# zivy/LSQRRecipes

Hardware: AMD Instinct MI355X
Metric: RANSAC hypotheses/sec + final-fit residual, 10M pts, 1/2/4/8 GPU (higher is better)
Workload: dtype f64; 1 GPU; PlaneParametersEstimator + RANSAC, 10000000 points, 50% outliers, delta=0.50 (BASELINE.json configs[1]); points=10000000, streams=4, world_size=1, collectives=none (single GPU), repeats=3

## Files before the change

### lsqrrecipes_amd/csrc/cells.h

```cpp
#pragma once
#include <hip/hip_runtime.h>
#include <stdint.h>

#include "models.h"

#pragma clang diagnostic ignored "-Winline-asm"

namespace lsqr {

constexpr int kCellPtsMin = 128;
constexpr uint32_t kGroupPad = 4, kCellPad = 16;
constexpr uint32_t kQueues = 32;
constexpr uint32_t kQueuePitch = 1088;

struct CellBox {
  float c[3];
  float h[3];
  float pad[2];
};

__device__ inline unsigned long long ord_u64(double v) {
  unsigned long long b;
  __builtin_memcpy(&b, &v, 8);
  return (b >> 63) ? ~b : (b | 0x8000000000000000ULL);
}
inline double ord_u64_inv(unsigned long long o) {
  unsigned long long b = (o >> 63) ? (o & 0x7FFFFFFFFFFFFFFFULL) : ~o;
  double v;
  memcpy(&v, &b, 8);
  return v;
}

struct BoundsRow {
  unsigned long long mn[3], mx[3], amax, nonfinite;
};
template <int D>
__global__ __launch_bounds__(256) void k_bounds(const double *__restrict__ data, size_t stride,
                                                size_t n, BoundsRow *__restrict__ rows) {
  unsigned long long mn[D], mx[D], am = 0, bad = 0;
  for (int d = 0; d < D; d++) mn[d] = ~0ULL, mx[d] = 0ULL;
  auto one = [&](const double(&x)[D]) {
    bool fin = true;
    for (int d = 0; d < D; d++) fin = fin && (fabs(x[d]) <= 1.7976931348623157e308);
    if (!fin) {
// ... 780 lines not shown
  static __device__ inline v2f value(const v2f *xs, const v2f *fp) {
    return M::filter_value(xs, fp);
  }
};
template <int D>
inline CellConsts cell_consts(const LineCell<D> *, const ModelConsts &mc) {
  const double u = 5.9604644775390625e-08, s3 = 1.7320508075688774;
  const double rc = 2.0 * mc.delta, cap = 4.0 * mc.delta_sq;
  const double eta = 1e-12 * 2.0 * mc.absmax;
  CellConsts cc;
  memset(&cc, 0, sizeof cc);
  cc.f[0] = f32_down_host(mc.delta_sq);
  cc.f[1] = f32_up_host(mc.delta_sq);
  cc.f[2] = f32_up_host(6.0 * u * (1.0 + 4.0 * u) * (1.0 + 1e-6));
  cc.f[3] = f32_up_host((u * rc + 2.0 * eta) * (1.0 + 1e-6));
  cc.f[4] = f32_up_host(2.0 * s3 * rc * (1.0 + 1e-6));
  cc.f[5] = f32_up_host(4.0 * u * cap * (1.0 + 1e-6));
  cc.f[6] = f32_down_host(0.25 * mc.delta / (6.0 * s3 * u) * (1.0 - 1e-6));
  cc.f[7] = f32_down_host(0.25 * mc.delta_sq * (1.0 - 1e-6));
  return cc;
}

template <int NB>
__device__ __forceinline__ void cells_filter_squares(float (&bc)[NB]) {
  const float tin = bc[NB - 2], tout = bc[NB - 1];
  const bool off = !(tout < __builtin_inff());
  const float a = tin > 0.0f ? (tin * tin) * 0.9999998f : 0.0f;
  const float c = (tout * tout) * 1.0000002f;
  const float band = c - a;
  bc[NB - 2] = off ? 0.0f : a;
  bc[NB - 1] = off ? __builtin_bit_cast(float, 0xFFFFFFFFu) : band;
}

template <class CM, int PP, bool LDSB, bool DUP = false>
__device__ __forceinline__ void cells_survivors(const v2f (&xs)[PP][4], const float (&bc)[CM::NB], float *s_bc,
                                                unsigned long long surv, const int lane,
                                                const double *__restrict__ sorted, const size_t ns, const size_t cell,
                                                const double *__restrict__ spg, const ModelConsts &mc,
                                                uint32_t &accv) {
  typedef typename CM::M M;
  constexpr int D = M::ND, NB = CM::NB, NV = CM::NV, SPD = M::SP, CP = 128 * PP;
  (void)D, (void)NV, (void)CP;
  if (LDSB && surv) {
    float4 w0, w1;
    if constexpr (DUP) {
      static_assert(LDSB && NB == 6 && NV == 4, "slots: fp0 fp1 fp3 fp3 | a a fp2 band");
      w0.x = bc[0], w0.y = bc[1], w0.z = bc[3], w0.w = bc[3];
      w1.x = bc[4], w1.y = bc[4], w1.z = bc[2], w1.w = bc[5];
    } else {
      w0.x = bc[0], w0.y = NB > 1 ? bc[1 < NB ? 1 : 0] : 0.0f, w0.z = NB > 2 ? bc[2 < NB ? 2 : 0] : 0.0f,
      w0.w = NB > 3 ? bc[3 < NB ? 3 : 0] : 0.0f;
      w1.x = NB > 4 ? bc[4 < NB ? 4 : 0] : 0.0f, w1.y = NB > 5 ? bc[5 < NB ? 5 : 0] : 0.0f,
      w1.z = NB > 6 ? bc[6 < NB ? 6 : 0] : 0.0f, w1.w = NB > 7 ? bc[7 < NB ? 7 : 0] : 0.0f;
    }
    ((float4 *)s_bc)[2 * lane] = w0;
    ((float4 *)s_bc)[2 * lane + 1] = w1;
  }
  while (surv) {
    const int b = __builtin_ctzll(surv);
    asm("s_bitset0_b64 %0, %1" : "+s"(surv) : "s"(b));
    v2f fp[NV], na;
    uint32_t band;
    if constexpr (DUP) {
      const float4 r0 = ((const float4 *)s_bc)[2 * b], r1 = ((const float4 *)s_bc)[2 * b + 1];
      fp[0].x = r0.x, fp[0].y = r0.x, fp[1].x = r0.y, fp[1].y = r0.y, fp[2].x = r1.z, fp[2].y = r1.z;
      fp[3].x = r0.z, fp[3].y = r0.w;
      na.x = -r1.x, na.y = -r1.y;
      band = __builtin_bit_cast(uint32_t, r1.w);
    } else if (LDSB) {
      static_assert(NB <= 8, "broadcast area holds 8 floats per lane");
      const float4 r0 = ((const float4 *)s_bc)[2 * b], r1 = ((const float4 *)s_bc)[2 * b + 1];
      const float rb[8] = {r0.x, r0.y, r0.z, r0.w, r1.x, r1.y, r1.z, r1.w};
// ... 2 lines not shown
      na.x = -rb[NB - 2], na.y = -rb[NB - 2];
      band = __builtin_bit_cast(uint32_t, rb[NB - 1]);
    } else {
#pragma unroll
      for (int k = 0; k < NV; k++) {
        float v = __builtin_bit_cast(
            float, __builtin_amdgcn_readlane(__builtin_bit_cast(int, bc[k]), b));
        fp[k].x = v;
        fp[k].y = v;
      }
      const float a = __builtin_bit_cast(float, __builtin_amdgcn_readlane(__builtin_bit_cast(int, bc[NB - 2]), b));
      na.x = -a, na.y = -a;
      band = (uint32_t)__builtin_amdgcn_readlane(__builtin_bit_cast(int, bc[NB - 1]), b);
    }
    unsigned long long in[2 * PP];
    uint32_t dmin = 0;
    v2f sv[PP];
#pragma unroll
    for (int p = 0; p < PP; p++) sv[p] = CM::value(xs[p], fp);
#pragma unroll
    for (int p = 0; p < PP; p++) {
      const v2f s = sv[p];
      const v2f d = __builtin_elementwise_fma(s, s, na);
      in[2 * p] = __ballot(d.x < 0.0f);
      in[2 * p + 1] = __ballot(d.y < 0.0f);
      typedef uint32_t v2u __attribute__((ext_vector_type(2)));
      const v2u du = __builtin_bit_cast(v2u, d);
      const uint32_t m = du.x < du.y ? du.x : du.y;
      dmin = p == 0 ? m : (m < dmin ? m : dmin);
    }
    const unsigned long long amb = __ballot(dmin <= band);
    if (amb) {
      const double *hp = spg + (size_t)b * SPD;
#pragma unroll
      for (int p = 0; p < PP; p++) {
        const size_t i0 = cell * CP + p * 128 + lane, i1 = i0 + 64;
        double r0[D], r1[D];
#pragma unroll
        for (int d = 0; d < D; d++) {
          r0[d] = i0 < ns ? sorted[i0 * D + d] : __builtin_nan("");
          r1[d] = i1 < ns ? sorted[i1 * D + d] : __builtin_nan("");
        }
        in[2 * p] = __ballot(M::agree(hp, r0, mc));
        in[2 * p + 1] = __ballot(M::agree(hp, r1, mc));
      }
    }
    uint32_t cnt = 0;
#pragma unroll
    for (int p = 0; p < 2 * PP; p++) cnt += (uint32_t)__builtin_popcountll(in[p]);
    asm volatile("s_mov_b32 m0, %2\n\tv_writelane_b32 %0, %1, m0"
                 : "+v"(accv)
                 : "s"(cnt), "s"(b)
                 : "m0");
  }
}

template <class CM, int PP>
__device__ __forceinline__ void cells_load(const double *__restrict__ sorted, const size_t ns, const size_t cell,
                                           const int lane, const double (&ctr)[3], v2f (&xs)[PP][4]) {
  constexpr int D = CM::M::ND, CP = 128 * PP;
#pragma unroll
  for (int p = 0; p < PP; p++) {
    const size_t i0 = cell * CP + p * 128 + lane, i1 = i0 + 64;
    const double *p0 = sorted + (i0 < ns ? i0 : 0) * D, *p1 = sorted + (i1 < ns ? i1 : 0) * D;
#pragma unroll
    for (int d = 0; d < 3; d++) {
// ... 323 lines not shown
  const uint32_t h = blockIdx.x * 256 + threadIdx.x;
  if (h >= cap) return;
  float row[ROW], row2[NR2 ? 4 * NR2 : 4];
  const float4 *r4 = (const float4 *)(rows + (size_t)(h < H ? h : 0) * ROW);
#pragma unroll
  for (int k = 0; k < NR4; k++) {
    const float4 v = r4[k];
    row[4 * k] = v.x, row[4 * k + 1] = v.y, row[4 * k + 2] = v.z, row[4 * k + 3] = v.w;
  }
  if constexpr (NR2 > 0) {
    const float4 *q4 = (const float4 *)(spf + (size_t)(h < H ? h : 0) * M::SPF + CM::ROW2_OFF);
#pragma unroll
    for (int k = 0; k < NR2; k++) {
      const float4 v = q4[k];
      row2[4 * k] = v.x, row2[4 * k + 1] = v.y, row2[4 * k + 2] = v.z, row2[4 * k + 3] = v.w;
    }
  }
  typename CM::Hyp hy;
  CM::prepare(row, row2, h < H, cc, hy);
  const HypWords<CM> hw = __builtin_bit_cast(HypWords<CM>, hy);
#pragma unroll
  for (int k = 0; k < NH4; k++)
    out[(size_t)h * NH4 + k] = make_float4(hw.w[4 * k], hw.w[4 * k + 1], hw.w[4 * k + 2], hw.w[4 * k + 3]);
}
template <class CM>
__device__ __forceinline__ typename CM::Hyp hyp_from(const float4 (&v)[HypWords<CM>::N4]) {
  HypWords<CM> hw;
#pragma unroll
  for (int k = 0; k < HypWords<CM>::N4; k++)
    hw.w[4 * k] = v[k].x, hw.w[4 * k + 1] = v[k].y, hw.w[4 * k + 2] = v[k].z, hw.w[4 * k + 3] = v[k].w;
  return __builtin_bit_cast(typename CM::Hyp, hw);
}

template <class CM, int PP, bool PREP = false, bool COUNT = false>
__global__ __launch_bounds__(256) void k_cells_bounds(const CellBox *__restrict__ boxes, uint32_t ncells,
                                                      size_t ns, const float *__restrict__ rows,
                                                      const float *__restrict__ spf, uint32_t H,
                                                      CellConsts cc, uint32_t cells_per_block,
                                                      uint32_t *__restrict__ ub,
                                                      unsigned long long *__restrict__ total,
                                                      uint32_t *__restrict__ ncells_out,
                                                      uint8_t *__restrict__ cnt, uint32_t gstride,
                                                      const uint32_t *__restrict__ h_dev, uint32_t h_off,
                                                      uint32_t box_pop, const float4 *__restrict__ hyps) {
  typedef typename CM::M M;
  constexpr int ROW = CM::ROW, NR4 = ROW / 4, NR2 = CM::ROW2 / 4;
  const size_t CP = box_pop;
  const int lane = threadIdx.x & 63;
  if (h_dev) {
    const uint32_t hd = *h_dev > h_off ? *h_dev - h_off : 0u;
    H = hd < H ? hd : H;
  }
  const uint32_t grp = COUNT ? blockIdx.y * 4 + (uint32_t)__builtin_amdgcn_readfirstlane((int)(threadIdx.x >> 6))
                             : blockIdx.y * 4 + (threadIdx.x >> 6);
  const uint32_t h = grp * 64 + lane;
  if (blockIdx.y * 256 >= H) return;
  const bool active = h - lane < H;
  typename CM::Hyp hy;
  if constexpr (PREP) {
    constexpr int NH4 = HypWords<CM>::N4;
    float4 v[NH4];
#pragma unroll
    for (int k = 0; k < NH4; k++) v[k] = hyps[(size_t)(active ? h : 0) * NH4 + k];
    hy = hyp_from<CM>(v);
  } else {
    float row[ROW], row2[NR2 ? 4 * NR2 : 4];
    {
// ... 1 lines not shown
#pragma unroll
      for (int k = 0; k < NR4; k++) {
        const float4 v = r4[k];
        row[4 * k] = v.x, row[4 * k + 1] = v.y, row[4 * k + 2] = v.z, row[4 * k + 3] = v.w;
      }
      if constexpr (NR2 > 0) {
        const float4 *q4 = (const float4 *)(spf + (size_t)(h < H ? h : 0) * M::SPF + CM::ROW2_OFF);
#pragma unroll
        for (int k = 0; k < NR2; k++) {
          const float4 v = q4[k];
          row2[4 * k] = v.x, row2[4 * k + 1] = v.y, row2[4 * k + 2] = v.z, row2[4 * k + 3] = v.w;
        }
      }
    }
    CM::load(row, row2, h < H, cc, hy);
  }
  const uint32_t c0 = blockIdx.x * cells_per_block;
  const uint32_t c1 = c0 + cells_per_block < ncells ? c0 + cells_per_block : ncells;
  uint32_t u = 0, nc = 0;
  constexpr uint32_t BCH = 128;
  __shared__ CellBox s_box[BCH];
  __shared__ double s_ctr[BCH][3];
  for (uint32_t cb = c0; cb < c1; cb += BCH) {
    const uint32_t n = c1 - cb < BCH ? c1 - cb : BCH;
    __syncthreads();
    if (threadIdx.x < 2 * n) ((float4 *)s_box)[threadIdx.x] = ((const float4 *)(boxes + cb))[threadIdx.x];
    __syncthreads();
    if (threadIdx.x < n) {
#pragma unroll
      for (int d = 0; d < 3; d++) s_ctr[threadIdx.x][d] = (double)s_box[threadIdx.x].c[d];
    }
    __syncthreads();
    if (!active) continue;
    if constexpr (COUNT) {
      auto padded = [&](const CellBox &bx, const double (&ctr)[3]) {
        float bc[CM::NB];
        const uint32_t pc = (uint32_t)__builtin_popcountll(__ballot(CM::level1(hy, bx, ctr, cc, bc)));
        return (uint8_t)(pc ? pc + kGroupPad : 0u);
      };
      uint8_t *p = cnt + ((size_t)cb * gstride + grp);
      uint32_t i = 0;
      for (; i + 4 <= n; i += 4, p += 4 * gstride) {
        const CellBox b0 = s_box[i], b1 = s_box[i + 1], b2 = s_box[i + 2], b3 = s_box[i + 3];
        const double t0[3] = {s_ctr[i][0], s_ctr[i][1], s_ctr[i][2]};
        const double t1[3] = {s_ctr[i + 1][0], s_ctr[i + 1][1], s_ctr[i + 1][2]};
        const double t2[3] = {s_ctr[i + 2][0], s_ctr[i + 2][1], s_ctr[i + 2][2]};
        const double t3[3] = {s_ctr[i + 3][0], s_ctr[i + 3][1], s_ctr[i + 3][2]};
        const uint8_t p0 = padded(b0, t0), p1 = padded(b1, t1), p2 = padded(b2, t2), p3 = padded(b3, t3);
        if (lane == 0) p[0] = p0, p[gstride] = p1, p[2 * gstride] = p2, p[3 * gstride] = p3;
      }
      for (; i < n; i++, p += gstride) {
        const CellBox b0 = s_box[i];
        const double t0[3] = {s_ctr[i][0], s_ctr[i][1], s_ctr[i][2]};
        const uint8_t p0 = padded(b0, t0);
        if (lane == 0) p[0] = p0;
      }
      continue;
    }
    auto one = [&](const uint32_t i, const CellBox &bx, const double (&ctr)[3]) {
      const uint32_t c = cb + i;
      float bc[CM::NB];
      const bool s = CM::level1(hy, bx, ctr, cc, bc);
      const size_t first = (size_t)c * CP;
      const uint32_t pop = first + CP <= ns ? (uint32_t)CP : (uint32_t)(ns - first);
      u += s ? pop : 0u;
      nc += s ? 1u : 0u;
      if (cnt) {
        const uint32_t pc = (uint32_t)__builtin_popcountll(__ballot(s));
        if (lane == 0) cnt[(size_t)c * gstride + grp] = (uint8_t)(pc ? pc + kGroupPad : 0u);
      }
    };
    uint32_t i = 0;
    for (; i + 4 <= n; i += 4) {
      const CellBox b0 = s_box[i], b1 = s_box[i + 1], b2 = s_box[i + 2], b3 = s_box[i + 3];
      const double t0[3] = {s_ctr[i][0], s_ctr[i][1], s_ctr[i][2]};
      const double t1[3] = {s_ctr[i + 1][0], s_ctr[i + 1][1], s_ctr[i + 1][2]};
      const double t2[3] = {s_ctr[i + 2][0], s_ctr[i + 2][1], s_ctr[i + 2][2]};
      const double t3[3] = {s_ctr[i + 3][0], s_ctr[i + 3][1], s_ctr[i + 3][2]};
      one(i, b0, t0);
      one(i + 1, b1, t1);
      one(i + 2, b2, t2);
      one(i + 3, b3, t3);
    }
    for (; i < n; i++) {
      const CellBox b0 = s_box[i];
      const double t0[3] = {s_ctr[i][0], s_ctr[i][1], s_ctr[i][2]};
      one(i, b0, t0);
    }
  }
  if constexpr (COUNT) return;
  if (ub && h < H && u) atomicAdd(&ub[h], u);
  if (ncells_out && h < H && nc) atomicAdd(&ncells_out[h], nc);
  if (total) {
    for (int o = 32; o > 0; o >>= 1) nc += __shfl_down(nc, o);
    if (lane == 0 && nc) atomicAdd(total, (unsigned long long)nc);
  }
}

constexpr uint32_t kChunkCells = 128;

__global__ __launch_bounds__(128) void k_tile_costs(const uint8_t *__restrict__ cnt, uint32_t gstride, uint32_t H,
                                                    const uint32_t *__restrict__ h_dev, uint32_t ncells,
                                                    uint32_t *__restrict__ cost, uint32_t *__restrict__ csum,
                                                    uint32_t *__restrict__ votes, uint32_t h_off) {
  for (uint32_t i = blockIdx.x * kChunkCells + threadIdx.x; i < H; i += gridDim.x * kChunkCells) votes[i] = 0;
  if (h_dev) {
    const uint32_t hd = *h_dev > h_off ? *h_dev - h_off : 0u;
    H = hd < H ? hd : H;
  }
  const uint32_t G = (H + 63) / 64;
  const uint32_t c = blockIdx.x * kChunkCells + threadIdx.x;
  uint32_t t = 0;
  if (c < ncells) {
    const uint8_t *p = cnt + (size_t)c * gstride;
    uint32_t g = 0;
    if ((gstride & 15u) == 0)
      for (; g + 16 <= G; g += 16) {
        const uint4 v = *(const uint4 *)(p + g);
        t += __builtin_amdgcn_sad_u8(v.x, 0u, 0u) + __builtin_amdgcn_sad_u8(v.y, 0u, 0u) +
             __builtin_amdgcn_sad_u8(v.z, 0u, 0u) + __builtin_amdgcn_sad_u8(v.w, 0u, 0u);
      }
    for (; g < G; g++) t += p[g];
    t = t ? t + kCellPad : 0u;
    cost[c] = t;
  }
  __shared__ uint32_t s_w[2];
  for (int o = 32; o > 0; o >>= 1) t += __shfl_down(t, o);
  if ((threadIdx.x & 63) == 0) s_w[threadIdx.x >> 6] = t;
  __syncthreads();
  if (threadIdx.x == 0) csum[blockIdx.x] = s_w[0] + s_w[1];
}

__device__ __forceinline__ uint32_t wave_incl_scan(uint32_t v, int lane) {
#pragma unroll
  for (int o = 1; o < 64; o <<= 1) {
    const uint32_t a = __shfl_up(v, o);
    v += lane >= o ? a : 0u;
  }
  return v;
}

template <class CM, int PP, int BS, bool LDSB, bool PREP = false, bool LEAN = false>
__global__ __launch_bounds__(BS) __attribute__((amdgpu_waves_per_eu(PP >= 8 ? 4 : CM::MIN_WAVES, 8))) void k_scan_pairs(
    const double *__restrict__ sorted, size_t ns, const CellBox *__restrict__ boxes, uint32_t ncells,
    const double *__restrict__ sp, const float *__restrict__ rows, const float *__restrict__ spf, uint32_t H,
    ModelConsts mc, CellConsts cc, uint32_t *__restrict__ vpart, uint32_t vstride,
    const uint32_t *__restrict__ h_dev, const uint8_t *__restrict__ cnt, uint32_t gstride, const uint32_t *__restrict__ cost,
    const uint32_t *__restrict__ csum, uint32_t nchunks, uint32_t h_off, const float4 *__restrict__ hyps) {
  typedef typename CM::M M;
  constexpr int NB = CM::NB;
  constexpr int SPD = M::SP;
  [[maybe_unused]] constexpr int ROW = CM::ROW;
  constexpr int NR2 = CM::ROW2 / 4;
  constexpr int NR4 = [] {
    if constexpr (PREP) return (int)HypWords<CM>::N4;
    else return (int)CM::ROW / 4;
  }();
  if (h_dev) {
    const uint32_t hd = *h_dev > h_off ? *h_dev - h_off : 0u;
    H = hd < H ? hd : H;
  }
  extern __shared__ uint32_t s_cnt[];
  for (uint32_t h = threadIdx.x; h < H; h += BS) s_cnt[h] = 0;
  __syncthreads();
  const int lane = threadIdx.x & 63;
  float *s_bc = (float *)(s_cnt + ((H + 3) & ~3u)) + (size_t)(threadIdx.x >> 6) * 512;
  const uint32_t W = gridDim.x * (BS / 64);
  const uint32_t wid = blockIdx.x * (BS / 64) + (uint32_t)__builtin_amdgcn_readfirstlane((int)(threadIdx.x >> 6));

  unsigned long long C = 0;
  for (uint32_t k0 = 0; k0 < nchunks; k0 += 64) {
    uint32_t v = k0 + lane < nchunks ? csum[k0 + lane] : 0u;
    for (int o = 32; o > 0; o >>= 1) v += __shfl_xor(v, o);
    C += (uint32_t)__builtin_amdgcn_readfirstlane((int)v);
  }
  const unsigned long long t0 = C * wid / W, t1 = C * (wid + 1) / W;
  uint32_t budget = (uint32_t)(t1 - t0);
  uint32_t cell = ncells, skip = 0;
  if (budget) {
    unsigned long long base = 0;
    uint32_t chunk = 0;
    for (uint32_t k0 = 0; k0 < nchunks; k0 += 64) {
      const uint32_t v = k0 + lane < nchunks ? csum[k0 + lane] : 0u;
      const uint32_t inc = wave_incl_scan(v, lane);
      const uint32_t tot = (uint32_t)__builtin_amdgcn_readlane((int)inc, 63);
      if (base + tot > t0) {
        const unsigned long long hit = __ballot(base + inc > t0);
        const int l = __builtin_ctzll(hit);
        chunk = k0 + l;
        base += (uint32_t)__builtin_amdgcn_readlane((int)(inc - v), l);
        break;
      }
      base += tot;
    }
    const uint32_t cb = chunk * kChunkCells + 2 * lane;
    const uint32_t v0 = cb < ncells ? cost[cb] : 0u, v1 = cb + 1 < ncells ? cost[cb + 1] : 0u;
    const uint32_t inc = wave_incl_scan(v0 + v1, lane);
    const uint32_t r = (uint32_t)(t0 - base);
    const unsigned long long hit = __ballot(inc > r);
    const int l = hit ? __builtin_ctzll(hit) : 63;
    const uint32_t before = (uint32_t)__builtin_amdgcn_readlane((int)(inc - v0 - v1), l);
// ... 5 lines not shown

  if constexpr (LEAN) {
    budget = (uint32_t)__builtin_amdgcn_readfirstlane((int)budget);
    cell = (uint32_t)__builtin_amdgcn_readfirstlane((int)cell);
    skip = (uint32_t)__builtin_amdgcn_readfirstlane((int)skip);
  }
  const uint32_t G = (H + 63) / 64;
  auto pad = [&](uint32_t P) {
    if (skip >= P) {
      skip -= P;
    } else {
      const uint32_t take = P - skip < budget ? P - skip : budget;
      budget -= take;
      skip = 0;
    }
  };
  auto load_rows = [&](uint32_t g, float4(&r)[NR4], float4(&r2)[NR2 ? NR2 : 1]) {
    const uint32_t h = g * 64 + lane;
    if constexpr (PREP) {
#pragma unroll
      for (int k = 0; k < NR4; k++) r[k] = hyps[(size_t)h * NR4 + k];
    } else {
      const float4 *r4 = (const float4 *)(rows + (size_t)(h < H ? h : 0) * ROW);
#pragma unroll
      for (int k = 0; k < NR4; k++) r[k] = r4[k];
      if constexpr (NR2 > 0) {
        const float4 *q4 = (const float4 *)(spf + (size_t)(h < H ? h : 0) * M::SPF + CM::ROW2_OFF);
#pragma unroll
        for (int k = 0; k < NR2; k++) r2[k] = q4[k];
      }
    }
  };
  while (budget && cell < ncells) {
    {
      const uint32_t v = cell + lane < ncells ? cost[cell + lane] : 0u;
      const unsigned long long nz = __ballot(v != 0);
      if (!nz) {
        cell += 64;
        continue;
      }
      cell += (uint32_t)__builtin_ctzll(nz);
    }
    pad(kCellPad);
    const uint32_t gc = (uint32_t)lane < G ? (uint32_t)cnt[(size_t)cell * gstride + lane] : 0u;
    unsigned long long gm = __ballot(gc != 0);
    while (gm && budget) {
      const int g = __builtin_ctzll(gm);
      const uint32_t cg = (uint32_t)__builtin_amdgcn_readlane((int)gc, g);
      if (skip < cg) break;
      skip -= cg;
      gm &= gm - 1;
    }
    if (!gm || !budget) {
      cell++;
      continue;
    }
    const CellBox bx = boxes[cell];
    double ctr[3];
#pragma unroll
    for (int d = 0; d < 3; d++) ctr[d] = (double)bx.c[d];
    if constexpr (LEAN && PP >= 4) {
#pragma unroll
      for (int d = 0; d < 3; d++) {
        const unsigned long long u = __builtin_bit_cast(unsigned long long, ctr[d]);
        uint32_t l, m;
        asm("s_nop 0\n\tv_readfirstlane_b32 %0, %1\n\ts_nop 1" : "=s"(l) : "v"((uint32_t)u));
        asm("s_nop 0\n\tv_readfirstlane_b32 %0, %1\n\ts_nop 1" : "=s"(m) : "v"((uint32_t)(u >> 32)));
        ctr[d] = __builtin_bit_cast(double, (unsigned long long)m << 32 | l);
      }
    }
    v2f xs[PP][4];
    cells_load<CM, PP>(sorted, ns, (size_t)cell, lane, ctr, xs);
    if constexpr (LEAN) {
      static_assert(PREP, "the lean group loop is built for prepared hypotheses");
      typename CM::Hyp hy;
      {
        float4 r[NR4], r2[1];
        load_rows((uint32_t)__builtin_ctzll(gm), r, r2);
        hy = hyp_from<CM>(r);
      }
      while (gm && budget) {
        const int g = __builtin_ctzll(gm);
        gm &= gm - 1;
        const uint32_t cg = (uint32_t)__builtin_amdgcn_readlane((int)gc, g);
        const uint32_t lo = skip, hi = cg < skip + budget ? cg : skip + budget;
        budget -= hi - lo;
        skip = 0;
        const uint32_t klo = lo > kGroupPad ? lo : kGroupPad;
        const bool mine = hi > klo;
        const uint32_t h0 = (uint32_t)g * 64, h = h0 + lane;
        float bc[NB];
        unsigned long long surv = 0;
        if (mine) surv = __ballot(CM::level1(hy, bx, ctr, cc, bc));
        if (gm) {
          float4 r[NR4], r2[1];
          load_rows((uint32_t)__builtin_ctzll(gm), r, r2);
          hy = hyp_from<CM>(r);
        }
        if (!mine) continue;
        cells_filter_squares(bc);
        for (uint32_t k = kGroupPad; k < lo; k++) surv &= surv - 1;
        if (hi < cg) {
          unsigned long long keep = 0, m = surv;
          for (uint32_t k = klo; k < hi; k++) {
            keep |= m & (0ull - m);
// ... 143 lines not shown
```

### lsqrrecipes_amd/csrc/lsqr_hip.hip

```cpp
#include <hip/hip_runtime.h>

#include <algorithm>
#include <atomic>
#include <chrono>
#include <cmath>
#include <cstdarg>
#include <cstddef>
#include <cstdio>
#include <cstdlib>
#include <cstring>
#include <limits>
#include <set>
#include <thread>
#include <string>
#include <type_traits>
#include <utility>
#include <vector>

#include "../../include/lsqr_hip.h"
#include "devbuf.h"
#include "kernels.h"
#include "models_nd.h"
#include "dense.h"
#include "dense_h16.h"
// ... 144 lines not shown
  bool us16_valid = false, us16_attr = false, us16_nomem = false;
  Us16Scales us16_sc{};
  int opt_us_h16 = 1;
  int opt_dense_fast = 1;
  int opt_us_fast = 1;
  DevBuf<uint8_t> d_refused;
  int opt_phantom_fast = 1;
  int opt_lm_tiles = 1;
  int opt_us_mask_mfma = 1;
  int opt_refine = 1;
  int opt_kd_levels = 7;
  int opt_kd_after = 16384;
  int kd_build_levels = 0, index_kd_levels = 0;
  int opt_presorted = 0;
  int opt_dense_wave = 3;
  int opt_dense_dd = 1;
  DevBuf<double> d_ddpart;
  int opt_index = 1, opt_cpt = 0, opt_cell = 0, opt_block = 0, opt_hsplit = 0, opt_pairs = 0, opt_pairs_waves = 0;
  DevBuf<uint8_t> d_valid;
  DevBuf<uint32_t> d_votes;
  DevBuf<uint32_t> d_ub;
  DevBuf<CellAxis> d_axis;
  DevBuf<float> d_cellT;
  bool axis_valid = false;
  int opt_mom_chunk = 0;
  int opt_hyp_order = 1;
  int opt_axis = 1;
  DevBuf<uint32_t> d_ub2;
  DevBuf<uint8_t> d_paircnt;
  DevBuf<uint32_t> d_paircost;
  DevBuf<uint32_t> d_vpart;
  DevBuf<float4> d_hyps;
  int opt_lean = 1;
  int opt_prepared = 1;
  DevBuf<uint32_t> d_sel;
  DevBuf<BoundSel> d_bsel;
  DevBuf<double> d_hparams2;
  DevBuf<float> d_hparams2_f32;
  DevBuf<uint32_t> d_votes2;
  int opt_bound = 1;
  uint32_t best_before = 0;
  bool allow_bound = false;
  uint64_t last_bound[4] = {0, 0, 0, 0};
  DevBuf<char> d_ee;
  PinBuf<EeState> h_ee;
  bool ee_last = false;
  uint64_t ee_H = 0, ee_n = 0;
  bool scanned = false;
  bool external_stream = false;
  static constexpr int kMaxLanes = 4;
  lsqr_ctx *lanes[kMaxLanes] = {nullptr, nullptr, nullptr, nullptr};
  int opt_lanes = 4;
  bool is_lane = false;
  uint64_t data_epoch = 1;
  uint64_t lane_epoch = 0;
  std::vector<std::pair<std::string, int>> opt_log;
  Event slot_ev[2];
  bool defer_ovf = false;
  uint32_t ovf_cap = 0;
  uint32_t slot_ovf_cap[2] = {0, 0};
  uint64_t slot_seed[2] = {0, 0};
  int opt_test_overflow = 0;
  uint64_t ovf_reruns = 0;
  uint64_t slot_first[2] = {0, 0}, slot_H[2] = {0, 0};
  bool slot_busy[2] = {false, false};
  Event mdev_ev[4];
// ... 715 lines not shown
      ScanBatch sub = {b0.sp + h0 * M::SP, b0.spf + h0 * M::SPF, std::min<size_t>(kPairsChunk, b0.H - h0),
                       b0.votes + h0, b0.h_dev, (uint32_t)(b0.h_off + h0)};
      int st = run_scan_pairs<CM, PP>(c, sub);
      if (st != LSQR_OK) return st;
    }
    return LSQR_OK;
  }
  const ScanBatch &b = b0;
  const CellConsts cc = cell_consts((const CM *)nullptr, c->mc);
  if (c->n_cells == 0 || b.H == 0) {
    HIPCHK(c, hipMemsetAsync(b.votes, 0, b.H * sizeof(uint32_t), c->stream));
    return LSQR_OK;
  }
  const uint32_t Hc = (uint32_t)b.H, groups = (Hc + 63) / 64;
  const uint32_t gstride = groups <= 1 ? 1u : (groups + 15) / 16 * 16;
  const uint32_t nchunks = (c->n_cells + kChunkCells - 1) / kChunkCells;
  int st;
  if ((st = ensure(c, c->d_paircnt, (size_t)c->n_cells * gstride)) != LSQR_OK) return st;
  if ((st = ensure(c, c->d_paircost, (size_t)c->n_cells + nchunks)) != LSQR_OK) return st;
  uint32_t *d_cost = c->d_paircost, *d_csum = c->d_paircost + c->n_cells;
  const float *rows = CM::ROW_F32 ? b.spf : (const float *)b.sp;
  constexpr bool kPrep = cell_prepared<CM>();
  const bool prep = kPrep && c->opt_prepared;
  if constexpr (kPrep) {
    if (prep) {
      const uint32_t slots = (Hc + 63) & ~63u;
      if ((st = ensure(c, c->d_hyps, (size_t)slots * HypWords<CM>::N4)) != LSQR_OK) return st;
      hipLaunchKernelGGL((k_prepare_hyps<CM>), dim3((slots + 255) / 256), dim3(256), 0, c->stream, rows, b.spf, Hc, cc,
                         b.h_dev, b.h_off, c->d_hyps);
      HIPCHK(c, hipGetLastError());
    }
  }
  const float4 *hyps = prep ? c->d_hyps : nullptr;
  {
    const unsigned gy = (Hc + 255) / 256;
    const uint32_t per = std::max<uint32_t>(8, (c->n_cells + 1023) / 1024);
    const unsigned gx = (c->n_cells + per - 1) / per;
    auto count = [&](auto kern) {
      hipLaunchKernelGGL(kern, dim3(gx, gy), dim3(256), 0, c->stream, c->d_boxes, c->n_cells, c->n_sorted, rows, b.spf,
                         Hc, cc, per, (uint32_t *)nullptr, (unsigned long long *)nullptr, (uint32_t *)nullptr,
                         c->d_paircnt, gstride, b.h_dev, b.h_off, (uint32_t)(128 * PP), hyps);
    };
    if (c->opt_lean) {
      if (prep)
        count(k_cells_bounds<CM, PP, kPrep, true>);
      else
        count(k_cells_bounds<CM, PP, false, true>);
    } else if (prep)
      count(k_cells_bounds<CM, PP, kPrep>);
    else
      count(k_cells_bounds<CM, PP>);
    HIPCHK(c, hipGetLastError());
  }
  hipLaunchKernelGGL(k_tile_costs, dim3(nchunks), dim3(kChunkCells), 0, c->stream, c->d_paircnt, gstride, Hc, b.h_dev,
                     c->n_cells, d_cost, d_csum, b.votes, b.h_off);
  HIPCHK(c, hipGetLastError());
  bool ldsb_default = CM::LDS_BROADCAST;
  if constexpr (requires { CM::LDS_BROADCAST_PAIRS; }) ldsb_default = CM::LDS_BROADCAST_PAIRS;
  const bool ldsb = c->opt_block == 257 || (c->opt_block == 0 && ldsb_default);
  constexpr int BS = 256, wpb = BS / 64;
  const size_t lds = (size_t)((Hc + 3) & ~3u) * sizeof(uint32_t) + (ldsb ? (size_t)wpb * 2048 : 0);
  auto launch = [&](auto kern) -> int {
    int per_cu = (int)std::min<size_t>(32 / wpb, (160 * 1024) / std::max<size_t>(lds, 1)), occ = 0;
    if (hipOccupancyMaxActiveBlocksPerMultiprocessor(&occ, kern, BS, lds) == hipSuccess && occ >= 1)
      per_cu = std::min(per_cu, occ);
    else
      (void)hipGetLastError();
    if (per_cu < 1) per_cu = 1;
    if (c->opt_pairs_waves > 0) per_cu = std::min(per_cu, c->opt_pairs_waves);
    const unsigned blocks = (unsigned)std::min<size_t>(((size_t)c->n_cells + wpb - 1) / wpb, (size_t)256 * per_cu);
    int st2 = ensure(c, c->d_vpart, (size_t)blocks * Hc);
    if (st2 != LSQR_OK) return st2;
    ProfScope ps(c, KID_SCAN);
    hipLaunchKernelGGL(kern, dim3(blocks), dim3(BS), lds, c->stream, c->d_sorted, c->n_sorted, c->d_boxes, c->n_cells,
                       b.sp, rows, b.spf, Hc, c->mc, cc, c->d_vpart, Hc, b.h_dev, (const uint8_t *)c->d_paircnt, gstride,
                       (const uint32_t *)d_cost, (const uint32_t *)d_csum, nchunks, b.h_off, hyps);
    HIPCHK(c, hipGetLastError());
    hipLaunchKernelGGL(k_votes_reduce, dim3((Hc + 63) / 64, 48), dim3(256), 0, c->stream,
                       (const uint32_t *)c->d_vpart, Hc, (uint32_t)blocks, Hc, b.h_dev, b.votes, b.h_off);
    HIPCHK(c, hipGetLastError());
    return LSQR_OK;
  };
  if constexpr (kPrep) {
    if (prep && c->opt_lean)
      return ldsb ? launch(k_scan_pairs<CM, PP, BS, true, true, true>) : launch(k_scan_pairs<CM, PP, BS, false, true, true>);
  }
  if (prep) return ldsb ? launch(k_scan_pairs<CM, PP, BS, true, kPrep>) : launch(k_scan_pairs<CM, PP, BS, false, kPrep>);
  return ldsb ? launch(k_scan_pairs<CM, PP, BS, true>) : launch(k_scan_pairs<CM, PP, BS, false>);
}

template <int PP>
int run_rank_bounds(lsqr_ctx *c, const uint32_t **lo_out) {
  typedef PlaneCell<3> CM;
  typedef typename CM::M M;
  const uint32_t H = (uint32_t)c->H;
  int st;
  if (!c->d_ub2) HIPCHK(c, c->d_ub2.alloc(3 * c->H_cap));
  uint32_t *ub2 = c->d_ub2, *lb2 = c->d_ub2 + c->H_cap, *lo = c->d_ub2 + 2 * c->H_cap;
  const CellConsts cc = cell_consts((const CM *)nullptr, c->mc);
  uint32_t *cand = c->d_sel + kPilots;
  double *sp_b = c->d_hparams2 + (size_t)kPilots * M::SP;
  float *spf_b = c->d_hparams2_f32 + (size_t)kPilots * M::SPF;
  hipLaunchKernelGGL(k_pick_cands, dim3(1), dim3(1024), 0, c->stream, c->d_ub, c->d_valid, H, c->best_before, cand,
                     c->d_bsel, c->d_votes, ub2, lb2, lo);
  hipLaunchKernelGGL(k_gather_rows, dim3((H + 3) / 4), dim3(256), 0, c->stream, cand, &c->d_bsel->n_cand, H,
                     c->d_hparams, (int)M::SP, c->d_hparams_f32, (int)M::SPF, sp_b, spf_b);
  HIPCHK(c, hipGetLastError());
  const unsigned gy = (H + 511) / 512;
  const uint32_t per = std::max<uint32_t>(8, ((c->n_cells + 3071) / 3072 + 7) / 8 * 8);
  const unsigned gx = (c->n_cells + per - 1) / per;
  float thr_up = (float)c->mc.thr, thr_dn = thr_up;
  if ((double)thr_up < c->mc.thr) thr_up = nextafterf(thr_up, INFINITY);
  if ((double)thr_dn > c->mc.thr) thr_dn = nextafterf(thr_dn, -INFINITY);
  float xabs = (float)c->mc.absmax;
  if ((double)xabs < c->mc.absmax) xabs = nextafterf(xabs, INFINITY);
  hipLaunchKernelGGL((k_bound_axis<PP>), dim3(gx, gy), dim3(512), 0, c->stream, c->d_boxes, c->d_axis, c->d_cellT,
// ... 3735 lines not shown
  }
  if (!strcmp(name, "lm_host")) {
    c->opt_lm_host = value != 0;
    return LSQR_OK;
  }
  if (!strcmp(name, "scan_index")) {
    if (value < 0 || value > 2) return fail(c, LSQR_ERR_INVALID, "scan_index must be 0, 1 or 2");
    c->opt_index = value;
    return LSQR_OK;
  }
  if (!strcmp(name, "scan_cpt")) {
    if (value != 0 && value != 1) return fail(c, LSQR_ERR_INVALID, "scan_cpt must be 0 or 1");
    c->opt_cpt = value;
    return LSQR_OK;
  }
  if (!strcmp(name, "scan_bound_merge")) {
    if (value != 0 && value != 1 && value != 2 && value != 4 && value != 8)
      return fail(c, LSQR_ERR_INVALID, "scan_bound_merge must be 0, 1, 2, 4 or 8");
    c->opt_bound_merge = value;
    return LSQR_OK;
  }
  if (!strcmp(name, "scan_pairs")) {
    c->opt_pairs = value;
    return LSQR_OK;
  }
  if (!strcmp(name, "scan_prepared")) {
    c->opt_prepared = value != 0;
    return LSQR_OK;
  }
  if (!strcmp(name, "scan_lean")) {
    c->opt_lean = value != 0;
    return LSQR_OK;
  }
  if (!strcmp(name, "scan_axis")) {
    c->opt_axis = value != 0;
    return LSQR_OK;
  }
  if (!strcmp(name, "scan_hyp_order")) {
    c->opt_hyp_order = value != 0;
    return LSQR_OK;
  }
  if (!strcmp(name, "mom_chunk")) {
    c->opt_mom_chunk = value;
    return LSQR_OK;
  }
  if (!strcmp(name, "us_mfma")) {
    c->opt_us_h16 = value != 0;
    return LSQR_OK;
  }
  if (!strcmp(name, "scan_pairs_mfma")) {
    return value == 0 ? LSQR_OK : fail(c, LSQR_ERR_INVALID, "scan_pairs_mfma: removed (measured slower; tools/attic/cells_h16.h)");
  }
  if (!strcmp(name, "scan_pairs_waves")) {
    c->opt_pairs_waves = value;
    return LSQR_OK;
  }
  if (!strcmp(name, "scan_hsplit")) {
    if (value < 0 || value > 128) return fail(c, LSQR_ERR_INVALID, "scan_hsplit must be 0..128");
    c->opt_hsplit = value;
    return LSQR_OK;
  }
  if (!strcmp(name, "dense_mask_ring")) {
    c->opt_mask_ring = value;
    return LSQR_OK;
  }
  if (!strcmp(name, "dense_mask_diag")) {
// ... 238 lines not shown
```

Baseline: 6.284 million hypotheses/s.

## Pack surviving hypotheses per cell into dense 64-wide blocks via ballot masks

The count pass now writes a 64-bit survivor mask per hypothesis group and cell instead of a padded byte count. The pair scan compacts surviving hypothesis ids into LDS lists, using a DPP prefix scan and mbcnt, and processes full 64-lane blocks of gathered prepared hypotheses. The aim is to stop wasting lanes on sparsely populated groups and to even out per-cell cost. In exchange it adds mask storage eight times the size of the byte counts, extra LDS per wave, and index gather and compaction overhead. It is enabled by default when prepared lean mode is on.

```diff
diff --git a/lsqrrecipes_amd/csrc/cells.h b/lsqrrecipes_amd/csrc/cells.h
--- a/lsqrrecipes_amd/csrc/cells.h
+++ b/lsqrrecipes_amd/csrc/cells.h
@@ -10,6 +10,7 @@
 
 constexpr int kCellPtsMin = 128;
 constexpr uint32_t kGroupPad = 4, kCellPad = 16;
+constexpr uint32_t kBlockPad = 6;
 constexpr uint32_t kQueues = 32;
 constexpr uint32_t kQueuePitch = 1088;
 
@@ -856,12 +857,12 @@
   bc[NB - 1] = off ? __builtin_bit_cast(float, 0xFFFFFFFFu) : band;
 }
 
-template <class CM, int PP, bool LDSB, bool DUP = false>
+template <class CM, int PP, bool LDSB, bool DUP = false, bool PACKED = false>
 __device__ __forceinline__ void cells_survivors(const v2f (&xs)[PP][4], const float (&bc)[CM::NB], float *s_bc,
                                                 unsigned long long surv, const int lane,
                                                 const double *__restrict__ sorted, const size_t ns, const size_t cell,
                                                 const double *__restrict__ spg, const ModelConsts &mc,
-                                                uint32_t &accv) {
+                                                uint32_t &accv, const uint16_t *ids = nullptr) {
   typedef typename CM::M M;
   constexpr int D = M::ND, NB = CM::NB, NV = CM::NV, SPD = M::SP, CP = 128 * PP;
   (void)D, (void)NV, (void)CP;
@@ -930,6 +931,7 @@
     const unsigned long long amb = __ballot(dmin <= band);
     if (amb) {
       const double *hp = spg + (size_t)b * SPD;
+      if constexpr (PACKED) hp = spg + (size_t)(uint32_t)__builtin_amdgcn_readfirstlane((int)ids[b]) * SPD;
 #pragma unroll
       for (int p = 0; p < PP; p++) {
         const size_t i0 = cell * CP + p * 128 + lane, i1 = i0 + 64;
@@ -1319,7 +1321,7 @@
   return __builtin_bit_cast(typename CM::Hyp, hw);
 }
 
-template <class CM, int PP, bool PREP = false, bool COUNT = false>
+template <class CM, int PP, bool PREP = false, bool COUNT = false, bool MASK = false>
 __global__ __launch_bounds__(256) void k_cells_bounds(const CellBox *__restrict__ boxes, uint32_t ncells,
                                                       size_t ns, const float *__restrict__ rows,
                                                       const float *__restrict__ spf, uint32_t H,
@@ -1387,6 +1389,31 @@
     }
     __syncthreads();
     if (!active) continue;
+    if constexpr (MASK) {
+      static_assert(COUNT, "the masks are written by the count-only form");
+      auto mask = [&](const CellBox &bx, const double (&ctr)[3]) {
+        float bc[CM::NB];
+        return (unsigned long long)__ballot(CM::level1(hy, bx, ctr, cc, bc));
+      };
+      unsigned long long *p = (unsigned long long *)cnt + ((size_t)cb * gstride + grp);
+      uint32_t i = 0;
+      for (; i + 4 <= n; i += 4, p += 4 * gstride) {
+        const CellBox b0 = s_box[i], b1 = s_box[i + 1], b2 = s_box[i + 2], b3 = s_box[i + 3];
+        const double t0[3] = {s_ctr[i][0], s_ctr[i][1], s_ctr[i][2]};
+        const double t1[3] = {s_ctr[i + 1][0], s_ctr[i + 1][1], s_ctr[i + 1][2]};
+        const double t2[3] = {s_ctr[i + 2][0], s_ctr[i + 2][1], s_ctr[i + 2][2]};
+        const double t3[3] = {s_ctr[i + 3][0], s_ctr[i + 3][1], s_ctr[i + 3][2]};
+        const unsigned long long m0 = mask(b0, t0), m1 = mask(b1, t1), m2 = mask(b2, t2), m3 = mask(b3, t3);
+        if (lane == 0) p[0] = m0, p[gstride] = m1, p[2 * gstride] = m2, p[3 * gstride] = m3;
+      }
+      for (; i < n; i++, p += gstride) {
+        const CellBox b0 = s_box[i];
+        const double t0[3] = {s_ctr[i][0], s_ctr[i][1], s_ctr[i][2]};
+        const unsigned long long m0 = mask(b0, t0);
+        if (lane == 0) p[0] = m0;
+      }
+      continue;
+    }
     if constexpr (COUNT) {
       auto padded = [&](const CellBox &bx, const double (&ctr)[3]) {
         float bc[CM::NB];
@@ -1453,7 +1480,24 @@
 }
 
 constexpr uint32_t kChunkCells = 128;
-
+__host__ __device__ constexpr uint32_t pack_cell_cost(uint32_t S) {
+  return S ? kCellPad + (S + 63) / 64 * kBlockPad + S : 0u;
+}
+__host__ __device__ constexpr uint32_t pack_first(uint32_t u) {
+  const uint32_t v = u > kCellPad ? u - kCellPad : 0u, B = 64 + kBlockPad, q = v / B, r = v - q * B;
+  return 64 * q + (r > kBlockPad ? r - kBlockPad : 0u);
+}
+__host__ __device__ constexpr uint32_t pack_cell_survivors(uint32_t c) {
+  const uint32_t x = c - kCellPad, B = 64 + kBlockPad;
+  return x - (x + B - 1) / B * kBlockPad;
+}
+static_assert(pack_cell_survivors(pack_cell_cost(1)) == 1 && pack_cell_survivors(pack_cell_cost(64)) == 64 &&
+              pack_cell_survivors(pack_cell_cost(65)) == 65 && pack_cell_survivors(pack_cell_cost(4096)) == 4096);
+static_assert(pack_first(0) == 0 && pack_first(kCellPad + kBlockPad) == 0 && pack_first(kCellPad + kBlockPad + 1) == 1 &&
+              pack_first(kCellPad + kBlockPad + 64) == 64 && pack_first(kCellPad + 2 * kBlockPad + 64) == 64 &&
+              pack_first(kCellPad + 2 * kBlockPad + 65) == 65);
+
+template <bool PACK = false>
 __global__ __launch_bounds__(128) void k_tile_costs(const uint8_t *__restrict__ cnt, uint32_t gstride, uint32_t H,
                                                     const uint32_t *__restrict__ h_dev, uint32_t ncells,
                                                     uint32_t *__restrict__ cost, uint32_t *__restrict__ csum,
@@ -1466,7 +1510,19 @@
   const uint32_t G = (H + 63) / 64;
   const uint32_t c = blockIdx.x * kChunkCells + threadIdx.x;
   uint32_t t = 0;
-  if (c < ncells) {
+  if (PACK && c < ncells) {
+    const unsigned long long *p = (const unsigned long long *)cnt + (size_t)c * gstride;
+    uint32_t g = 0;
+    if ((gstride & 1u) == 0)
+      for (; g + 2 <= G; g += 2) {
+        const uint4 v = *(const uint4 *)(p + g);
+        t += (uint32_t)(__builtin_popcount(v.x) + __builtin_popcount(v.y) + __builtin_popcount(v.z) +
+                        __builtin_popcount(v.w));
+      }
+    for (; g < G; g++) t += (uint32_t)__builtin_popcountll(p[g]);
+    t = pack_cell_cost(t);
+    cost[c] = t;
+  } else if (c < ncells) {
     const uint8_t *p = cnt + (size_t)c * gstride;
     uint32_t g = 0;
     if ((gstride & 15u) == 0)
@@ -1495,7 +1551,17 @@
   return v;
 }
 
-template <class CM, int PP, int BS, bool LDSB, bool PREP = false, bool LEAN = false>
+__device__ __forceinline__ uint32_t wave_incl_scan_dpp(uint32_t v) {
+  v += (uint32_t)__builtin_amdgcn_update_dpp(0, (int)v, 0x111, 0xf, 0xf, false);
+  v += (uint32_t)__builtin_amdgcn_update_dpp(0, (int)v, 0x112, 0xf, 0xf, false);
+  v += (uint32_t)__builtin_amdgcn_update_dpp(0, (int)v, 0x114, 0xf, 0xf, false);
+  v += (uint32_t)__builtin_amdgcn_update_dpp(0, (int)v, 0x118, 0xf, 0xf, false);
+  v += (uint32_t)__builtin_amdgcn_update_dpp(0, (int)v, 0x142, 0xa, 0xf, false);
+  v += (uint32_t)__builtin_amdgcn_update_dpp(0, (int)v, 0x143, 0xc, 0xf, false);
+  return v;
+}
+
+template <class CM, int PP, int BS, bool LDSB, bool PREP = false, bool LEAN = false, bool PACK = false>
 __global__ __launch_bounds__(BS) __attribute__((amdgpu_waves_per_eu(PP >= 8 ? 4 : CM::MIN_WAVES, 8))) void k_scan_pairs(
     const double *__restrict__ sorted, size_t ns, const CellBox *__restrict__ boxes, uint32_t ncells,
     const double *__restrict__ sp, const float *__restrict__ rows, const float *__restrict__ spf, uint32_t H,
@@ -1522,6 +1588,13 @@
   float *s_bc = (float *)(s_cnt + ((H + 3) & ~3u)) + (size_t)(threadIdx.x >> 6) * 512;
   const uint32_t W = gridDim.x * (BS / 64);
   const uint32_t wid = blockIdx.x * (BS / 64) + (uint32_t)__builtin_amdgcn_readfirstlane((int)(threadIdx.x >> 6));
+  [[maybe_unused]] uint16_t *s_id = nullptr;
+  if constexpr (PACK) {
+    static_assert(LEAN && PREP, "packed blocks gather prepared hypotheses and run the lean pair loop");
+    s_id = (uint16_t *)((float *)(s_cnt + ((H + 3) & ~3u)) + (LDSB ? (size_t)(BS / 64) * 512 : 0)) +
+           (size_t)__builtin_amdgcn_readfirstlane((int)(threadIdx.x >> 6)) * 128;
+    s_id[lane] = 0, s_id[64 + lane] = 0;
+  }
 
   unsigned long long C = 0;
   for (uint32_t k0 = 0; k0 < nchunks; k0 += 64) {
@@ -1593,6 +1666,7 @@
     }
   };
   while (budget && cell < ncells) {
+    [[maybe_unused]] uint32_t ccost = 0;
     {
       const uint32_t v = cell + lane < ncells ? cost[cell + lane] : 0u;
       const unsigned long long nz = __ballot(v != 0);
@@ -1601,20 +1675,43 @@
         continue;
       }
       cell += (uint32_t)__builtin_ctzll(nz);
-    }
-    pad(kCellPad);
-    const uint32_t gc = (uint32_t)lane < G ? (uint32_t)cnt[(size_t)cell * gstride + lane] : 0u;
-    unsigned long long gm = __ballot(gc != 0);
-    while (gm && budget) {
-      const int g = __builtin_ctzll(gm);
-      const uint32_t cg = (uint32_t)__builtin_amdgcn_readlane((int)gc, g);
-      if (skip < cg) break;
-      skip -= cg;
-      gm &= gm - 1;
-    }
-    if (!gm || !budget) {
-      cell++;
-      continue;
+      if constexpr (PACK) ccost = (uint32_t)__builtin_amdgcn_readlane((int)v, __builtin_ctzll(nz));
+    }
+    [[maybe_unused]] uint32_t jlo = 0, jhi = 0;
+    uint32_t gc = 0;
+    unsigned long long gm = 0;
+    if constexpr (PACK) {
+      if (skip >= ccost) {
+        skip -= ccost;
+        cell++;
+        continue;
+      }
+      const uint32_t S = pack_cell_survivors(ccost);
+      const uint32_t lo = skip, hi = ccost < skip + budget ? ccost : skip + budget;
+      budget -= hi - lo;
+      skip = 0;
+      jlo = (uint32_t)__builtin_amdgcn_readfirstlane((int)pack_first(lo));
+      jhi = (uint32_t)__builtin_amdgcn_readfirstlane((int)pack_first(hi));
+      jhi = jhi < S ? jhi : S;
+      if (jhi <= jlo) {
+        cell++;
+        continue;
+      }
+    } else {
+      pad(kCellPad);
+      gc = (uint32_t)lane < G ? (uint32_t)cnt[(size_t)cell * gstride + lane] : 0u;
+      gm = __ballot(gc != 0);
+      while (gm && budget) {
+        const int g = __builtin_ctzll(gm);
+        const uint32_t cg = (uint32_t)__builtin_amdgcn_readlane((int)gc, g);
+        if (skip < cg) break;
+        skip -= cg;
+        gm &= gm - 1;
+      }
+      if (!gm || !budget) {
+        cell++;
+        continue;
+      }
     }
     const CellBox bx = boxes[cell];
     double ctr[3];
@@ -1632,6 +1729,58 @@
     }
     v2f xs[PP][4];
     cells_load<CM, PP>(sorted, ns, (size_t)cell, lane, ctr, xs);
+    if constexpr (PACK) {
+      const unsigned long long ra = (unsigned long long)cnt + ((unsigned long long)cell * gstride << 3);
+      const unsigned long long *row = (const unsigned long long *)(
+          (unsigned long long)(uint32_t)__builtin_amdgcn_readfirstlane((int)(uint32_t)(ra >> 32)) << 32 |
+          (uint32_t)__builtin_amdgcn_readfirstlane((int)(uint32_t)ra));
+      const unsigned long long pm = (uint32_t)lane < G ? row[(uint32_t)lane] : 0ull;
+      const uint32_t pc = (uint32_t)__builtin_popcountll(pm);
+      const uint32_t incl = wave_incl_scan_dpp(pc);
+      const uint32_t excl = pc ? incl - pc : ~0u;
+      auto block_ids = [&](const uint32_t base, uint16_t *list) {
+        const unsigned long long upto = __ballot(excl <= base);
+        unsigned long long ov = __ballot(excl < base + 64) & (~0ull << (63 - __builtin_clzll(upto)));
+        while (ov) {
+          const int g = __builtin_ctzll(ov);
+          ov &= ov - 1;
+          const uint32_t mlo = (uint32_t)__builtin_amdgcn_readlane((int)(uint32_t)pm, g),
+                         mhi = (uint32_t)__builtin_amdgcn_readlane((int)(uint32_t)(pm >> 32), g);
+          const uint32_t r = (uint32_t)__builtin_amdgcn_readlane((int)excl, g) - base;
+          const uint32_t slot = __builtin_amdgcn_mbcnt_hi(mhi, __builtin_amdgcn_mbcnt_lo(mlo, r));
+          if (__builtin_amdgcn_inverse_ballot_w64((unsigned long long)mhi << 32 | mlo) && slot < 64)
+            list[slot] = (uint16_t)((uint32_t)g * 64 + (uint32_t)lane);
+        }
+        __builtin_amdgcn_wave_barrier();
+        return (uint32_t)list[lane];
+      };
+      auto gather = [&](const uint32_t id) {
+        float4 r[NR4];
+#pragma unroll
+        for (int k = 0; k < NR4; k++) r[k] = hyps[(size_t)id * NR4 + k];
+        return hyp_from<CM>(r);
+      };
+      uint32_t base = jlo, par = 0;
+      typename CM::Hyp hy = gather(block_ids(base, s_id));
+      for (;;) {
+        const uint32_t n = jhi - base < 64 ? jhi - base : 64;
+        const unsigned long long surv = ~0ull >> (uint32_t)__builtin_amdgcn_readfirstlane((int)(64 - n));
+        float bc[NB];
+        (void)CM::level1(hy, bx, ctr, cc, bc);
+        base += 64;
+        const bool more = base < jhi;
+        if (more) hy = gather(block_ids(base, s_id + (par ^ 64)));
+        cells_filter_squares(bc);
+        uint32_t accv = 0;
+        cells_survivors<CM, PP, LDSB, LDSB, true>(xs, bc, s_bc, surv, lane, sorted, ns, (size_t)cell, sp, mc, accv,
+                                                  s_id + par);
+        if (accv) atomicAdd(&s_cnt[s_id[par + lane]], accv);
+        if (!more) break;
+        par ^= 64;
+      }
+      cell++;
+      continue;
+    }
     if constexpr (LEAN) {
       static_assert(PREP, "the lean group loop is built for prepared hypotheses");
       typename CM::Hyp hy;
diff --git a/lsqrrecipes_amd/csrc/lsqr_hip.hip b/lsqrrecipes_amd/csrc/lsqr_hip.hip
--- a/lsqrrecipes_amd/csrc/lsqr_hip.hip
+++ b/lsqrrecipes_amd/csrc/lsqr_hip.hip
@@ -200,6 +200,8 @@
   DevBuf<uint32_t> d_vpart;
   DevBuf<float4> d_hyps;
   int opt_lean = 1;
+  DevBuf<unsigned long long> d_pairmask;
+  int opt_pack = 1;
   int opt_prepared = 1;
   DevBuf<uint32_t> d_sel;
   DevBuf<BoundSel> d_bsel;
@@ -981,6 +983,9 @@
     }
   }
   const float4 *hyps = prep ? c->d_hyps : nullptr;
+  const bool pack = prep && c->opt_lean && c->opt_pack;
+  if (pack && (st = ensure(c, c->d_pairmask, (size_t)c->n_cells * gstride)) != LSQR_OK) return st;
+  uint8_t *d_cnt = pack ? (uint8_t *)c->d_pairmask.get() : c->d_paircnt.get();
   {
     const unsigned gy = (Hc + 255) / 256;
     const uint32_t per = std::max<uint32_t>(8, (c->n_cells + 1023) / 1024);
@@ -988,9 +993,11 @@
     auto count = [&](auto kern) {
       hipLaunchKernelGGL(kern, dim3(gx, gy), dim3(256), 0, c->stream, c->d_boxes, c->n_cells, c->n_sorted, rows, b.spf,
                          Hc, cc, per, (uint32_t *)nullptr, (unsigned long long *)nullptr, (uint32_t *)nullptr,
-                         c->d_paircnt, gstride, b.h_dev, b.h_off, (uint32_t)(128 * PP), hyps);
+                         d_cnt, gstride, b.h_dev, b.h_off, (uint32_t)(128 * PP), hyps);
     };
-    if (c->opt_lean) {
+    if (pack) {
+      if constexpr (kPrep) count(k_cells_bounds<CM, PP, true, true, true>);
+    } else if (c->opt_lean) {
       if (prep)
         count(k_cells_bounds<CM, PP, kPrep, true>);
       else
@@ -1001,14 +1008,21 @@
       count(k_cells_bounds<CM, PP>);
     HIPCHK(c, hipGetLastError());
   }
-  hipLaunchKernelGGL(k_tile_costs, dim3(nchunks), dim3(kChunkCells), 0, c->stream, c->d_paircnt, gstride, Hc, b.h_dev,
-                     c->n_cells, d_cost, d_csum, b.votes, b.h_off);
+  auto costs = [&](auto kern) {
+    hipLaunchKernelGGL(kern, dim3(nchunks), dim3(kChunkCells), 0, c->stream, (const uint8_t *)d_cnt, gstride, Hc,
+                       b.h_dev, c->n_cells, d_cost, d_csum, b.votes, b.h_off);
+  };
+  if (pack)
+    costs(k_tile_costs<true>);
+  else
+    costs(k_tile_costs<false>);
   HIPCHK(c, hipGetLastError());
   bool ldsb_default = CM::LDS_BROADCAST;
   if constexpr (requires { CM::LDS_BROADCAST_PAIRS; }) ldsb_default = CM::LDS_BROADCAST_PAIRS;
   const bool ldsb = c->opt_block == 257 || (c->opt_block == 0 && ldsb_default);
   constexpr int BS = 256, wpb = BS / 64;
-  const size_t lds = (size_t)((Hc + 3) & ~3u) * sizeof(uint32_t) + (ldsb ? (size_t)wpb * 2048 : 0);
+  const size_t lds = (size_t)((Hc + 3) & ~3u) * sizeof(uint32_t) + (ldsb ? (size_t)wpb * 2048 : 0) +
+                     (pack ? (size_t)wpb * 256 : 0);
   auto launch = [&](auto kern) -> int {
     int per_cu = (int)std::min<size_t>(32 / wpb, (160 * 1024) / std::max<size_t>(lds, 1)), occ = 0;
     if (hipOccupancyMaxActiveBlocksPerMultiprocessor(&occ, kern, BS, lds) == hipSuccess && occ >= 1)
@@ -1022,7 +1036,7 @@
     if (st2 != LSQR_OK) return st2;
     ProfScope ps(c, KID_SCAN);
     hipLaunchKernelGGL(kern, dim3(blocks), dim3(BS), lds, c->stream, c->d_sorted, c->n_sorted, c->d_boxes, c->n_cells,
-                       b.sp, rows, b.spf, Hc, c->mc, cc, c->d_vpart, Hc, b.h_dev, (const uint8_t *)c->d_paircnt, gstride,
+                       b.sp, rows, b.spf, Hc, c->mc, cc, c->d_vpart, Hc, b.h_dev, (const uint8_t *)d_cnt, gstride,
                        (const uint32_t *)d_cost, (const uint32_t *)d_csum, nchunks, b.h_off, hyps);
     HIPCHK(c, hipGetLastError());
     hipLaunchKernelGGL(k_votes_reduce, dim3((Hc + 63) / 64, 48), dim3(256), 0, c->stream,
@@ -1031,6 +1045,9 @@
     return LSQR_OK;
   };
   if constexpr (kPrep) {
+    if (pack)
+      return ldsb ? launch(k_scan_pairs<CM, PP, BS, true, true, true, true>)
+                  : launch(k_scan_pairs<CM, PP, BS, false, true, true, true>);
     if (prep && c->opt_lean)
       return ldsb ? launch(k_scan_pairs<CM, PP, BS, true, true, true>) : launch(k_scan_pairs<CM, PP, BS, false, true, true>);
   }
@@ -4832,6 +4849,11 @@
     c->opt_lean = value != 0;
     return LSQR_OK;
   }
+  if (!strcmp(name, "scan_pack")) {
+    if (value != 0 && value != 1) return fail(c, LSQR_ERR_INVALID, "scan_pack must be 0 or 1");
+    c->opt_pack = value;
+    return LSQR_OK;
+  }
   if (!strcmp(name, "scan_axis")) {
     c->opt_axis = value != 0;
     return LSQR_OK;
```

After: 6.621 million hypotheses/s, median of 6. 5.4% higher.
